# AllenNeuralDynamics/aind-exaspim-image-compression

Hardware: AMD Instinct MI355X
Metric: denoised+encoded voxels/s on 1024^3 uint16 (higher is better)
Workload: dtype f32

## Files before the change

aind-exaspim-image-compression_amd/csrc/stage_kernels.hip:

```cpp
#include <algorithm>
#include <type_traits>

#include "exabm4d_kernels.h"
#include "dct_pairs.h"
#ifdef EXABM4D_STAMPS
#define KERNEL_STAMPS
#endif
#include "kernel_stamps.h"

namespace exabm4d {

typedef float f16v __attribute__((ext_vector_type(16)));

#ifdef EXABM4D_STAMPS
__device__ unsigned long long g_stamps[18];
#endif

constexpr float HAAR_C = 0.70710678118654752440f;

__device__ __forceinline__ void gather8v(__amdgpu_buffer_rsrc_t rsrc, int corner, const unsigned (&voff)[8],
                                         float (&v)[8]) {
#pragma unroll
    for (int y = 0; y < 8; y++)
        v[y] = __int_as_float(__builtin_amdgcn_raw_buffer_load_b32(rsrc, (int)voff[y], corner, 0));
}

template <int K>
__device__ __forceinline__ void haar_fwd2(f2 (&v)[MAXG]) {
#pragma unroll
    for (int len = K; len > 1; len >>= 1) {
        const int half = len >> 1;
        f2 t[MAXG];
#pragma unroll
        for (int i = 0; i < half; i++) {
            t[i] = (v[2 * i] + v[2 * i + 1]) * HAAR_C;
            t[half + i] = (v[2 * i] - v[2 * i + 1]) * HAAR_C;
        }
#pragma unroll
        for (int i = 0; i < len; i++) v[i] = t[i];
    }
}
template <int K>
__device__ __forceinline__ void haar_inv2(f2 (&v)[MAXG]) {
#pragma unroll
    for (int len = 1; len < K; len <<= 1) {
        f2 t[MAXG];
#pragma unroll
        for (int i = 0; i < len; i++) {
            t[2 * i] = (v[i] + v[len + i]) * HAAR_C;
            t[2 * i + 1] = (v[i] - v[len + i]) * HAAR_C;
        }
#pragma unroll
        for (int i = 0; i < 2 * len; i++) v[i] = t[i];
    }
}

typedef unsigned u2v __attribute__((ext_vector_type(2)));
__device__ __forceinline__ void gather8v2(__amdgpu_buffer_rsrc_t rsrc, int corner2, const unsigned (&voff)[8],
                                          float (&a)[8], float (&b)[8]) {
#pragma unroll
    for (int y = 0; y < 8; y++) {
        const u2v t = __builtin_amdgcn_raw_buffer_load_b64(rsrc, (int)(2u * voff[y]), corner2, 0);
        a[y] = __uint_as_float(t.x);
        b[y] = __uint_as_float(t.y);
    }
}

struct TileGeom {
    int y0, x0;
    int nry, nrx;
};

#ifndef EXABM4D_HT_NW
#define EXABM4D_HT_NW 12
#endif
#ifndef EXABM4D_HT_TY
// ... 23 lines not shown
    static constexpr int TBW = 2 * TBUF;
    static constexpr int NW = NW_;
    static constexpr int TY = TY_, TX = TX_;
    static constexpr int ROWS = (TY - 1) * STEP + 18;
    static constexpr int COLS = (TX - 1) * STEP + 18;
    static constexpr int PS = ((ROWS * COLS + 23) / 32) * 32 + 8;
    static constexpr int NPL = NPL_;
    static constexpr size_t LDS_FLOATS = (size_t)2 * NPL * PS + (size_t)NW * TBW + 4 + 2 * NW + 8 + NW;
    static_assert(NW % 2 == 0 && NW <= 16 && NPL >= 18 && NPL <= 26, "pairs of waves; at most 3 layers in flight");
    static_assert(LDS_FLOATS * sizeof(float) <= 160 * 1024, "ring + transpose buffers exceed the CU's LDS");
};
template <bool WIENER>
struct HalfCfg : HalfGeom<EXABM4D_HT_NW, EXABM4D_HT_TY, EXABM4D_HT_TX, EXABM4D_HT_NPL> {};
template <>
struct HalfCfg<true> : HalfGeom<EXABM4D_WIE_NW, EXABM4D_WIE_TY, EXABM4D_WIE_TX, EXABM4D_WIE_NPL> {};
constexpr int HNCNT = 8;
typedef long long ring_t;
constexpr double RINT_MAGIC = 6755399441055744.0;
__device__ __forceinline__ long long magic_bits(double m) {
    const unsigned long long b = (unsigned long long)__double_as_longlong(m);
    const unsigned hi = (unsigned)(b >> 32) - 0x43380000u;
    return (long long)(((unsigned long long)hi << 32) | (b & 0xFFFFFFFFull));
}
#ifndef EXABM4D_WIE_ILV
#define EXABM4D_WIE_ILV 2
#endif
__device__ __forceinline__ f2 rcp_nr2(f2 d) {
    f2 r = mk2(__uint_as_float(0x7EF311C7u - __float_as_uint(d.x)), __uint_as_float(0x7EF311C7u - __float_as_uint(d.y)));
#pragma unroll
    for (int i = 0; i < 3; i++) r = __builtin_elementwise_fma(__builtin_elementwise_fma(-d, r, (f2)(1.0f)), r, r);
    return r;
}
__device__ __forceinline__ f2 wiener_w2(f2 e, float sigma2, unsigned& acc) {
    const f2 W = e * rcp_nr2(e + sigma2);
    const f2 q = __builtin_elementwise_fma(W, W, (f2)(1.0f));
    acc += __float_as_uint(q.x);
    acc += __float_as_uint(q.y);
    return W;
}
constexpr unsigned WSQ_BIAS = 2u * 0x3F800000u;

__device__ __forceinline__ void wait_flag(const int* flag, int want, int lane) {
    cbar();
    if (lane == 0) {
        while (__hip_atomic_load(flag, __ATOMIC_RELAXED, __HIP_MEMORY_SCOPE_WORKGROUP) < want)
            __builtin_amdgcn_s_sleep(4);
    }
    cbar();
}
__device__ __forceinline__ void raise_flag(int* flag, int value, int lane) {
    cbar();
    if (lane == 0) __hip_atomic_store(flag, value, __ATOMIC_RELAXED, __HIP_MEMORY_SCOPE_WORKGROUP);
    cbar();
}

template <int KH>
__device__ __forceinline__ void half_shrink_local(f16v (&S)[4], float thr, int& nnz, f2 (&approx)[4]) {
#pragma unroll
    for (int jp = 0; jp < 4; jp++) {
        f16v A = S[jp];
        f2 x[MAXG];
#pragma unroll
        for (int k = 0; k < KH; k++) x[k] = mk2(A[2 * k], A[2 * k + 1]);
        haar_fwd2<KH>(x);
        approx[jp] = x[0];
#pragma unroll
        for (int k = 1; k < KH; k++) {
            const bool k0 = fabsf(x[k].x) >= thr, k1 = fabsf(x[k].y) >= thr;
            nnz += (k0 ? 1 : 0) + (k1 ? 1 : 0);
            float f0 = k0 ? x[k].x : 0.0f, f1 = k1 ? x[k].y : 0.0f;
            asm volatile("" : "+v"(f0), "+v"(f1));
            A[2 * k] = f0;
            A[2 * k + 1] = f1;
        }
        S[jp] = A;
    }
}
template <int KH>
__device__ __forceinline__ void half_unshrink_local(f16v (&S)[4], const f2 (&approx)[4]) {
#pragma unroll
    for (int jp = 0; jp < 4; jp++) {
        f16v A = S[jp];
        f2 x[MAXG];
        x[0] = approx[jp];
#pragma unroll
        for (int k = 1; k < KH; k++) x[k] = mk2(A[2 * k], A[2 * k + 1]);
        haar_inv2<KH>(x);
#pragma unroll
        for (int k = 0; k < KH; k++) {
            A[2 * k] = x[k].x;
            A[2 * k + 1] = x[k].y;
        }
        S[jp] = A;
    }
}

template <class C>
__device__ __forceinline__ void flush_num_plane(ring_t* ring, long long* __restrict__ num, int z,
                                                const TileGeom& tg, const VolGeom& g, int lane) {
    constexpr int REG = C::COLS;
    ring_t* plane = ring + ((z + 5) % C::NPL) * C::PS;
    constexpr int N = C::ROWS * REG, U = 6;
    const long long e0 = ((long long)z * g.ny + tg.y0) * (long long)g.nx + tg.x0;
    char* const sbase = reinterpret_cast<char*>(num) + e0 * 8;
    constexpr int DQ = 64 / REG, DR = 64 % REG;
    const unsigned row_adj = 8u * (unsigned)(g.nx - REG);
    const unsigned step = 8u * (unsigned)(DQ * g.nx + DR);
    int rxx = lane;
    asm volatile("" : "+v"(rxx));
    unsigned boff = 8u * (unsigned)rxx;
    const int lane0 = rxx;
#pragma unroll
    for (int j = 1; j * REG < 64; j++) {
        const bool w = lane0 >= j * REG;
        rxx -= w ? REG : 0;
        boff += w ? row_adj : 0u;
// ... 24 lines not shown
    int w = lane == 0 ? __hip_atomic_load(lock + 2, __ATOMIC_RELAXED, __HIP_MEMORY_SCOPE_WORKGROUP) : 0;
    w = __builtin_amdgcn_readfirstlane(w);
    if ((w >> 16) == 0) return false;
    {
        const int izp = izb + (w >> 16) - 1;
        if ((w & 0xFFFF) >= grid_pos(izp + 1, g.az, g.nz) - grid_pos(izp, g.az, g.nz)) return false;
    }
    w = lane == 0 ? __hip_atomic_fetch_add(lock + 2, 1, __ATOMIC_RELAXED, __HIP_MEMORY_SCOPE_WORKGROUP) : 0;
    w = __builtin_amdgcn_readfirstlane(w);
    const int gen = w >> 16, i = w & 0xFFFF;
    if (gen == 0) return false;
    const int iz = izb + gen - 1;
    const int z0 = grid_pos(iz, g.az, g.nz), zn = grid_pos(iz + 1, g.az, g.nz);
    if (i >= zn - z0) return false;
    cbar();
    flush_num_plane<C>(ring, num, z0 - RAD + i, tg, g, lane);
    cbar();
    if (lane == 0) __hip_atomic_fetch_add(lock + 3, 1, __ATOMIC_RELAXED, __HIP_MEMORY_SCOPE_WORKGROUP);
    cbar();
    return true;
}

template <int KH>
__device__ __forceinline__ void wiener_half_local(f16v (&S)[4], const f16v (&SB)[4], float sigma2,
                                                  unsigned& sw, f2 (&approx)[8]) {
#pragma unroll
    for (int jp = 0; jp < 4; jp++) {
        f16v A = S[jp];
        const f16v B = SB[jp];
        f2 x[MAXG], y[MAXG];
#pragma unroll
        for (int k = 0; k < KH; k++) {
            x[k] = mk2(A[2 * k], A[2 * k + 1]);
            y[k] = mk2(B[2 * k], B[2 * k + 1]);
        }
        haar_fwd2<KH>(x);
        haar_fwd2<KH>(y);
        approx[jp] = x[0];
        approx[4 + jp] = y[0];
#pragma unroll
        for (int k = 1; k < KH; k++) {
            const f2 W = wiener_w2(y[k] * y[k], sigma2, sw);
            const f2 f = W * x[k];
            A[2 * k] = f.x;
            A[2 * k + 1] = f.y;
            if (EXABM4D_WIE_ILV && (k % EXABM4D_WIE_ILV) == 0) __builtin_amdgcn_sched_barrier(0);
        }
        S[jp] = A;
    }
}

template <bool WIENER, typename TableT>
__device__ __forceinline__ bool process_half_group(
    const float* __restrict__ noisy, const float* __restrict__ basic, const uint32_t* __restrict__ kk,
    int rz, int ry, int rx, const TileGeom& tg, size_t sy, size_t sz, const TableT& T,
    const float (&win)[8], const float* __restrict__ win_g, float thr, float sigma2, double up, ring_t* ring,
    unsigned long long* __restrict__ cvol, f2* tb,
    f2* partner_tb, int* lock, int* sync, int* cnt, int wave, int& seq, int& seen, int layer, int target,
    int lane, long long g_nvox, long long* __restrict__ num, const VolGeom& g, int izb,
    const f2* __restrict__ pair
#ifdef EXABM4D_STAMPS
    , unsigned long long (&st)[16]
#endif
    ) {
    using C = HalfCfg<WIENER>;
    constexpr int HNW = C::NW, HNPL = C::NPL, HPS = C::PS, REG = C::COLS;
    constexpr bool HELP_FLUSH = !WIENER;
    constexpr int NP = WIENER ? 8 : 4;
    const int hi = lane >> 3, lo = lane & 7;
    const int xl = tr_x<WIENER>(hi, lo);
    STAMP(t0);
    const int half = pair_half(wave), partner = wave ^ 1;
    const uint32_t mykey = lane < MAXG ? kk[lane] : KEY_EMPTY;
    const int count = __popcll(__ballot(mykey != KEY_EMPTY));
    int K = 1;
    while (K * 2 <= count) K *= 2;
    const int KH = K > 1 ? K / 2 : 1;
    const int kb = K > 1 ? half * KH : 0;
    const bool active = K > 1 || half == 0;

    int closer = 0;
    auto body = [&](auto KHc) {
        constexpr int KH = decltype(KHc)::value;
        f16v S[4];
        f16v SB[WIENER ? 4 : 1];
#pragma unroll
        for (int j = 0; j < 4; j++) S[j] = (f16v)(0.0f);
        if constexpr (WIENER) {
#pragma unroll
            for (int j = 0; j < 4; j++) SB[j] = (f16v)(0.0f);
        }

        int my_dz, my_dy, my_dx;
        code_to_disp(mykey & KEY_CMASK, my_dz, my_dy, my_dx);
        const unsigned long long my_corner =
            lane < MAXG ? (unsigned long long)(rz + my_dz) * sz +
                              (unsigned long long)(ry + my_dy) * sy + (unsigned long long)(rx + my_dx)
                        : 0ull;
        const int zb = max(rz - RAD, 0);
        const size_t win_off = (size_t)zb * sz;
        const size_t win_left = (size_t)g_nvox - win_off;
        const int win_bytes = (int)min(win_left * sizeof(float), (size_t)0x7FFFFFFFu * 2u);
        const __amdgpu_buffer_rsrc_t noisy_r = __builtin_amdgcn_make_buffer_rsrc(
            const_cast<float*>(noisy + win_off), 0, win_bytes, 0x00020000);
        const __amdgpu_buffer_rsrc_t basic_r = __builtin_amdgcn_make_buffer_rsrc(
            const_cast<float*>((WIENER ? basic : noisy) + win_off), 0, win_bytes, 0x00020000);
        const int my_rel = lane < MAXG ? (int)(4u * (unsigned)(my_corner - win_off)) : 0;
        auto corner_of = [&](int k) -> int { return __builtin_amdgcn_readlane(my_rel, k); };
        const __amdgpu_buffer_rsrc_t pair_r = __builtin_amdgcn_make_buffer_rsrc(
            const_cast<f2*>((WIENER && pair ? pair : reinterpret_cast<const f2*>(noisy)) + (WIENER && pair ? win_off : 0)), 0,
            (int)min(win_left * sizeof(f2), (size_t)0x7FFFFFFFu * 2u), 0x00020000);
        float a[8], b[8];
        f2 v2[8];
        unsigned voff[8];
#pragma unroll
        for (int y = 0; y < 8; y++)
            voff[y] = 4u * ((unsigned)hi * (unsigned)sz + (unsigned)y * (unsigned)sy + (unsigned)lo);
        if constexpr (!WIENER && KH >= 4) {
            float c[8], d[8];
            f2 w2[8];
            gather8v(noisy_r, corner_of(kb), voff, a);
            gather8v(noisy_r, corner_of(kb + 1), voff, b);
            gather8v(noisy_r, corner_of(kb + 2), voff, c);
            gather8v(noisy_r, corner_of(kb + 3), voff, d);
#pragma unroll
            for (int kl = 0; kl < KH; kl += 4) {
#pragma unroll
                for (int j = 0; j < 8; j++) {
                    v2[j] = mk2(a[j], b[j]);
                    w2[j] = mk2(c[j], d[j]);
                }
                if (kl + 4 < KH) {
                    gather8v(noisy_r, corner_of(kb + kl + 4), voff, a);
                    gather8v(noisy_r, corner_of(kb + kl + 5), voff, b);
                    gather8v(noisy_r, corner_of(kb + kl + 6), voff, c);
                    gather8v(noisy_r, corner_of(kb + kl + 7), voff, d);
                }
                pair_fwd_x2<WIENER>(T, tb, hi, lo, v2, w2);
#pragma unroll
                for (int j = 0; j < 8; j++) {
                    S[j >> 1][2 * kl + (j & 1)] = v2[j].x;
                    S[j >> 1][2 * kl + 2 + (j & 1)] = v2[j].y;
                    S[j >> 1][2 * kl + 4 + (j & 1)] = w2[j].x;
                    S[j >> 1][2 * kl + 6 + (j & 1)] = w2[j].y;
                }
            }
        } else if constexpr (!WIENER) {
            gather8v(noisy_r, corner_of(kb), voff, a);
            gather8v(noisy_r, corner_of(kb + (KH > 1 ? 1 : 0)), voff, b);
#pragma unroll
            for (int kl = 0; kl < KH; kl += 2) {
#pragma unroll
                for (int j = 0; j < 8; j++) v2[j] = mk2(a[j], b[j]);
                if (kl + 2 < KH) {
                    gather8v(noisy_r, corner_of(kb + kl + 2), voff, a);
                    gather8v(noisy_r, corner_of(kb + kl + 3), voff, b);
                }
                pair_fwd<WIENER>(T, tb, hi, lo, v2);
#pragma unroll
                for (int j = 0; j < 8; j++) S[j >> 1][2 * kl + (j & 1)] = v2[j].x;
                if constexpr (KH > 1) {
#pragma unroll
                    for (int j = 0; j < 8; j++) S[j >> 1][2 * kl + 2 + (j & 1)] = v2[j].y;
                }
            }
        } else if constexpr (KH == 1) {
            const size_t c0 = corner_of(kb);
            if (pair) {
                gather8v2(pair_r, 2 * (int)c0, voff, a, b);
            } else {
                gather8v(noisy_r, c0, voff, a);
                gather8v(basic_r, c0, voff, b);
            }
#pragma unroll
            for (int j = 0; j < 8; j++) v2[j] = mk2(a[j], b[j]);
            pair_fwd<WIENER>(T, tb, hi, lo, v2);
#pragma unroll
            for (int j = 0; j < 8; j++) {
                S[j >> 1][j & 1] = v2[j].x;
                SB[j >> 1][j & 1] = v2[j].y;
            }
        } else if (pair) {
            gather8v2(pair_r, 2 * corner_of(kb), voff, a, b);
#pragma unroll
            for (int kl = 0; kl < KH; kl++) {
#pragma unroll
                for (int j = 0; j < 8; j++) v2[j] = mk2(a[j], b[j]);
                if (kl + 1 < KH) gather8v2(pair_r, 2 * corner_of(kb + kl + 1), voff, a, b);
                pair_fwd<WIENER>(T, tb, hi, lo, v2);
#pragma unroll
                for (int j = 0; j < 8; j++) {
                    S[j >> 1][2 * kl + (j & 1)] = v2[j].x;
                    SB[j >> 1][2 * kl + (j & 1)] = v2[j].y;
                }
            }
        } else {
            gather8v(noisy_r, corner_of(kb), voff, a);
            gather8v(noisy_r, corner_of(kb + 1), voff, b);
#pragma unroll
            for (int kl = 0; kl < KH; kl += 2) {
#pragma unroll
                for (int j = 0; j < 8; j++) v2[j] = mk2(a[j], b[j]);
                gather8v(basic_r, corner_of(kb + kl), voff, a);
                gather8v(basic_r, corner_of(kb + kl + 1), voff, b);
                pair_fwd<WIENER>(T, tb, hi, lo, v2);
#pragma unroll
                for (int j = 0; j < 8; j++) {
                    S[j >> 1][2 * kl + (j & 1)] = v2[j].x;
                    S[j >> 1][2 * kl + 2 + (j & 1)] = v2[j].y;
                }
#pragma unroll
                for (int j = 0; j < 8; j++) v2[j] = mk2(a[j], b[j]);
                if (kl + 2 < KH) {
                    gather8v(noisy_r, corner_of(kb + kl + 2), voff, a);
                    gather8v(noisy_r, corner_of(kb + kl + 3), voff, b);
                }
                pair_fwd<WIENER>(T, tb, hi, lo, v2);
#pragma unroll
                for (int j = 0; j < 8; j++) {
                    SB[j >> 1][2 * kl + (j & 1)] = v2[j].x;
                    SB[j >> 1][2 * kl + 2 + (j & 1)] = v2[j].y;
                }
            }
        }

        STAMP(t1);
        STAMP_ADD(0, t0, t1);
        int nnz = 0;
        unsigned sw = 0;
        f2 approx[NP];
        if constexpr (WIENER)
            wiener_half_local<KH>(S, SB, sigma2, sw, approx);
        else
            half_shrink_local<KH>(S, thr, nnz, approx);
        f2 top[4];
        if (K > 1) {
            seq++;
#pragma unroll
            for (int jp = 0; jp < NP; jp++) tb[jp * 64 + lane] = approx[jp];
            tb[NP * 64 + lane] = mk2(__int_as_float(WIENER ? (int)sw : nnz), 0.0f);
            raise_flag(sync + wave, seq, lane);
            STAMP(te0);
            wait_flag(sync + partner, seq, lane);
            STAMP(te1);
            STAMP_ADD(2, te0, te1);
            f2 other[NP];
#pragma unroll
            for (int jp = 0; jp < NP; jp++) other[jp] = partner_tb[jp * 64 + lane];
            const float theirs = partner_tb[NP * 64 + lane].x;
            cbar();
            raise_flag(sync + HNW + wave, seq, lane);
            if constexpr (WIENER)
                sw += __float_as_uint(theirs);
            else
                nnz += __float_as_int(theirs);
#pragma unroll
            for (int jp = 0; jp < 4; jp++) {
                const f2 a0 = half ? other[jp] : approx[jp], a1 = half ? approx[jp] : other[jp];
                f2 t0 = (a0 + a1) * HAAR_C, t1 = (a0 - a1) * HAAR_C;
                if constexpr (WIENER) {
                    const f2 b0 = half ? other[4 + jp] : approx[4 + jp];
                    const f2 b1 = half ? approx[4 + jp] : other[4 + jp];
                    const f2 u0 = (b0 + b1) * HAAR_C, u1 = (b0 - b1) * HAAR_C;
                    const f2 W0 = wiener_w2(u0 * u0, sigma2, sw);
                    const f2 W1 = wiener_w2(u1 * u1, sigma2, sw);
                    t0 = W0 * t0;
                    t1 = W1 * t1;
                } else {
                    const bool p0 = fabsf(t0.x) >= thr, p1 = fabsf(t0.y) >= thr;
                    const bool q0 = fabsf(t1.x) >= thr, q1 = fabsf(t1.y) >= thr;
                    nnz += (p0 ? 1 : 0) + (p1 ? 1 : 0) + (q0 ? 1 : 0) + (q1 ? 1 : 0);
                    t0 = mk2(p0 ? t0.x : 0.0f, p1 ? t0.y : 0.0f);
                    t1 = mk2(q0 ? t1.x : 0.0f, q1 ? t1.y : 0.0f);
                }
                top[jp] = half ? (t0 - t1) * HAAR_C : (t0 + t1) * HAAR_C;
                if constexpr (WIENER) __builtin_amdgcn_sched_barrier(0);
            }
        } else {
#pragma unroll
            for (int jp = 0; jp < 4; jp++) {
                if constexpr (WIENER) {
                    const f2 W = wiener_w2(approx[4 + jp] * approx[4 + jp], sigma2, sw);
                    top[jp] = W * approx[jp];
                } else {
                    const bool p0 = fabsf(approx[jp].x) >= thr, p1 = fabsf(approx[jp].y) >= thr;
                    nnz += (p0 ? 1 : 0) + (p1 ? 1 : 0);
                    top[jp] = mk2(p0 ? approx[jp].x : 0.0f, p1 ? approx[jp].y : 0.0f);
                }
            }
        }
        half_unshrink_local<KH>(S, top);
        float w;
        if constexpr (WIENER) {
            sw -= (K > 1 ? 8u * (unsigned)(KH - 1) + 8u : 4u) * WSQ_BIAS;
            unsigned lo16 = sw & 0xFFFFu, hi16 = sw >> 16;
#pragma unroll
            for (int off = 32; off >= 1; off >>= 1) {
                lo16 += __shfl_xor(lo16, off);
                hi16 += __shfl_xor(hi16, off);
            }
            const double q = (double)hi16 * 65536.0 + (double)lo16;
            const float stat = (float)(q * (1.0 / 8388608.0));
            w = 1.0f / (stat > 1.0f ? stat : 1.0f);
        } else {
#pragma unroll
            for (int off = 32; off >= 1; off >>= 1) nnz += __shfl_xor(nnz, off);
            w = 1.0f / (float)(nnz > 1 ? nnz : 1);
        }
        double ww[8];
        if constexpr (WIENER) {
#pragma unroll
            for (int y = 0; y < 8; y++) ww[y] = (double)(w * win_g[(hi * 8 + y) * 8 + xl]) * up;
        } else {
#pragma unroll
// ... 42 lines not shown
                STAMP_ADD(3, tg0, tg1);
            }
        };
        STAMP(t3);
        STAMP_ADD(5, t2, t3);
        auto ring_off = [&](int k) -> int {
            int slot = __builtin_amdgcn_readlane(my_slot0, k) + hi;
            slot -= slot >= HNPL ? HNPL : 0;
            return slot * HPS + __builtin_amdgcn_readlane(my_yx, k) + xl;
        };
        auto ring_add = [&](int off, const f2 (&v)[8], int comp) {
#pragma unroll
            for (int y = 0; y < 8; y++)
                __hip_atomic_fetch_add(reinterpret_cast<unsigned long long*>(ring + off + y * REG),
                                       (unsigned long long)magic_bits(__builtin_fma((double)(comp ? v[y].y : v[y].x), ww[y], RINT_MAGIC)),
                                       __ATOMIC_RELAXED, __HIP_MEMORY_SCOPE_WORKGROUP);
        };
        if constexpr (KH >= 4) {
            f2 w2[8];
#pragma unroll
            for (int kl = 0; kl < KH; kl += 4) {
#pragma unroll
                for (int j = 0; j < 8; j++) {
                    v2[j] = mk2(S[j >> 1][2 * kl + (j & 1)], S[j >> 1][2 * kl + 2 + (j & 1)]);
                    w2[j] = mk2(S[j >> 1][2 * kl + 4 + (j & 1)], S[j >> 1][2 * kl + 6 + (j & 1)]);
                }
                pair_inv_x2<WIENER>(T, tb, hi, lo, v2, w2);
                STAMP(tl1);
                gate(kb + kl);
                ring_add(ring_off(kb + kl), v2, 0);
                gate(kb + kl + 1);
                ring_add(ring_off(kb + kl + 1), v2, 1);
                gate(kb + kl + 2);
                ring_add(ring_off(kb + kl + 2), w2, 0);
                gate(kb + kl + 3);
                ring_add(ring_off(kb + kl + 3), w2, 1);
                STAMP(tl2);
                STAMP_ADD(4, tl1, tl2);
            }
        } else {
#pragma unroll
            for (int kl = 0; kl < KH; kl += 2) {
                constexpr bool two = KH > 1;
                const int kl2 = two ? kl + 1 : kl;
#pragma unroll
                for (int j = 0; j < 8; j++)
                    v2[j] = mk2(S[j >> 1][2 * kl + (j & 1)], S[j >> 1][2 * kl2 + (j & 1)]);
                pair_inv<WIENER>(T, tb, hi, lo, v2);
                STAMP(tl1);
                gate(kb + kl);
                ring_add(ring_off(kb + kl), v2, 0);
                if constexpr (two) {
                    gate(kb + kl2);
                    ring_add(ring_off(kb + kl2), v2, 1);
                }
                STAMP(tl2);
                STAMP_ADD(4, tl1, tl2);
            }
        }
    };
    if (active) {
        switch (KH) {
            case 8: body(std::integral_constant<int, 8>{}); break;
            case 4: body(std::integral_constant<int, 4>{}); break;
            case 2: body(std::integral_constant<int, 2>{}); break;
            default: body(std::integral_constant<int, 1>{}); break;
        }
    }
    if (!active) {
        if (lane == 0) {
            while (__hip_atomic_load(lock + 1, __ATOMIC_RELAXED, __HIP_MEMORY_SCOPE_WORKGROUP) < layer - 2)
                __builtin_amdgcn_s_sleep(8);
        }
        cbar();
    }
    closer = (__hip_atomic_fetch_add(cnt + (layer & (HNCNT - 1)), lane == 0 ? 1 : 0, __ATOMIC_RELAXED,
                                     __HIP_MEMORY_SCOPE_WORKGROUP) + 1 == target) ? 1 : 0;
    return __builtin_amdgcn_readfirstlane(closer) != 0;
}

typedef Dct7 HalfTable;
template <bool WIENER>
__global__ __launch_bounds__(HalfCfg<WIENER>::NW * 64) void stage_half_kernel(
    const float* __restrict__ noisy_all, const float* __restrict__ basic_all,
    const uint32_t* __restrict__ keys_all, VolGeom g, HalfTable T, const float* __restrict__ win_g,
    float thr, float sigma2, const double* __restrict__ qscale, long long* __restrict__ num_all,
    unsigned long long* __restrict__ cvol_all, int tiles_x, int layers_per_chunk, const f2* __restrict__ pair_all,
    int strip) {
    using C = HalfCfg<WIENER>;
    constexpr int HNW = C::NW, HNPL = C::NPL, HPS = C::PS, HTY = C::TY, HTX = C::TX;
    extern __shared__ __align__(16) float lds[];
    ring_t* ring = reinterpret_cast<ring_t*>(lds);
    const int wave = __builtin_amdgcn_readfirstlane(threadIdx.x >> 6), lane = threadIdx.x & 63;
    f2* tb = reinterpret_cast<f2*>(lds + 2 * HNPL * HPS + wave * C::TBW);
    f2* partner_tb = reinterpret_cast<f2*>(lds + 2 * HNPL * HPS + (wave ^ 1) * C::TBW);
    int* lock = reinterpret_cast<int*>(lds + 2 * HNPL * HPS + HNW * C::TBW);
    int* sync = lock + 4;
    int* cnt = sync + 2 * HNW;
    int* pub = cnt + HNCNT;
    int* got = pub + HNW / 2;

    const size_t voff = (size_t)blockIdx.z * (size_t)g.nvox;
    const float* __restrict__ noisy = noisy_all + voff;
    const float* __restrict__ basic = WIENER ? basic_all + voff : nullptr;
    const f2* __restrict__ pair = (WIENER && pair_all) ? pair_all + voff : nullptr;
    long long* __restrict__ num = num_all + voff;
    unsigned long long* __restrict__ cvol = cvol_all + voff;
    const double up = qscale[2 * blockIdx.z];
    const uint32_t* __restrict__ keys = keys_all + (size_t)blockIdx.z * (size_t)g.nref * MAXG;
    const size_t sy = (size_t)g.nx, sz = (size_t)g.nx * (size_t)g.ny;

    const int tile = xcd_contiguous(blockIdx.x, gridDim.x);
    int ty, tx;
    if (strip) {
        const int tiles_y = (int)gridDim.x / tiles_x;
        const int sidx = tile / (strip * tiles_x), r = tile - sidx * (strip * tiles_x);
        const int h = min(strip, tiles_y - sidx * strip);
        tx = r / h;
        ty = sidx * strip + (r - tx * h);
    } else {
        ty = tile / tiles_x;
        tx = tile - ty * tiles_x;
    }
    const int iy0 = HTY * ty, ix0 = HTX * tx;
    TileGeom tg;
    tg.nry = min(HTY, g.gy - iy0);
    tg.nrx = min(HTX, g.gx - ix0);
    tg.y0 = grid_pos(iy0, g.ay, g.ny) - RAD;
// ... 47 lines not shown
            }
            t = __builtin_amdgcn_readfirstlane(t) - 1;
        }
        cbar();
        last = t + 1;
        STAMP(th1);
        STAMP_ADD(6, th0, th1);
        if (t >= total) break;
        const int layer = t / nrefs, r = t - layer * nrefs;
        const int iz = izb + layer;
        const int z0 = grid_pos(iz, g.az, g.nz);
        const int jy = r / tg.nrx, jx = r - jy * tg.nrx;
        const int iy = iy0 + jy, ix = ix0 + jx;
        const int ry = grid_pos(iy, g.ay, g.ny), rx = grid_pos(ix, g.ax, g.nx);
        const uint32_t* kk = keys + ((size_t)((size_t)iz * g.gy + iy) * g.gx + ix) * MAXG;
        {
            int f = __hip_atomic_load(lock + 1, __ATOMIC_RELAXED, __HIP_MEMORY_SCOPE_WORKGROUP);
            f = __builtin_amdgcn_readfirstlane(f);
            if (layer <= f)
                __builtin_amdgcn_s_setprio(1);
            else
                __builtin_amdgcn_s_setprio(0);
        }
        const bool closer = process_half_group<WIENER>(
            noisy, basic, kk, z0, ry, rx, tg, sy, sz, tab, win, win_g, thr, sigma2, up, ring, cvol, tb,
            partner_tb, lock, sync, cnt, wave, seq, seen, layer, 2 * nrefs, lane, g.nvox, num, g, izb, pair
#ifdef EXABM4D_STAMPS
            , st
#endif
        );
        if (closer) {
            STAMP(tc0);
            if (lane == 0)
                __hip_atomic_store(cnt + (layer & (HNCNT - 1)), 0, __ATOMIC_RELAXED,
                                   __HIP_MEMORY_SCOPE_WORKGROUP);
            if (lane == 0) {
                while (__hip_atomic_load(lock + 1, __ATOMIC_RELAXED,
                                         __HIP_MEMORY_SCOPE_WORKGROUP) != layer)
                    __builtin_amdgcn_s_sleep(2);
            }
            cbar();
            if (iz + 1 < ize) {
                const int zn = grid_pos(iz + 1, g.az, g.nz);
                if constexpr (!WIENER) {
                    if (lane == 0) {
                        __hip_atomic_store(lock + 3, 0, __ATOMIC_RELAXED, __HIP_MEMORY_SCOPE_WORKGROUP);
                        __hip_atomic_store(lock + 2, (layer + 1) << 16, __ATOMIC_RELAXED,
// ... 26 lines not shown
    }
#ifdef EXABM4D_STAMPS
    st[7] = stamp() - tk0;
    if (lane == 0)
        for (int i = 0; i < 9; i++) atomicAdd(&g_stamps[i + (WIENER ? 9 : 0)], st[i]);
#endif
}

__global__ __launch_bounds__(256) void interleave_pair_kernel(const float* __restrict__ a, const float* __restrict__ b,
                                                              f2* __restrict__ out, size_t n) {
    for (size_t i = ((size_t)blockIdx.x * 256 + threadIdx.x) * 4; i < n; i += (size_t)gridDim.x * 1024) {
        if (i + 4 <= n) {
            const f4 x = *reinterpret_cast<const f4*>(a + i), y = *reinterpret_cast<const f4*>(b + i);
            f4 lo, hi;
            lo.x = x.x; lo.y = y.x; lo.z = x.y; lo.w = y.y;
            hi.x = x.z; hi.y = y.z; hi.z = x.w; hi.w = y.w;
            *reinterpret_cast<f4*>(out + i) = lo;
            *reinterpret_cast<f4*>(out + i + 2) = hi;
        } else {
            for (size_t j = i; j < n; j++) out[j] = mk2(a[j], b[j]);
        }
    }
}
hipError_t launch_stage(const float* noisy, const float* basic, const uint32_t* keys,
                        const VolGeom& g, int batch, const float* dct64, const float* win_dev,
                        float thr, float sigma2, const double* qscale, long long* num,
                        unsigned long long* cw, hipStream_t stream, const StageOpts& opt, float* pair,
                        int pair_ready) {
    DctTable T;
    for (int i = 0; i < 64; i++) T.d[i] = dct64[i];
    const size_t n = (size_t)g.nvox * (size_t)batch;
    Dct7 HT;
    if (!make_dct7(T, HT)) return hipErrorInvalidValue;
    auto launch = [&](auto wiener_c) -> hipError_t {
        constexpr bool W = decltype(wiener_c)::value;
        using C = HalfCfg<W>;
        if (((unsigned long long)(C::ROWS - 1) * (unsigned long long)g.nx + C::COLS) * 8ull > 0xFFFFFFFFull)
            return hipErrorInvalidValue;
        const int hty =(g.gy + C::TY - 1) / C::TY, htx = (g.gx + C::TX - 1) / C::TX;
        const long long htiles = (long long)hty * htx * batch;
        int hchunks = (int)((1024 + htiles - 1) / htiles);
        const int fine = (int)std::min<long long>((32768 + htiles - 1) / htiles, g.gz / 16);
        if (hchunks < fine) hchunks = fine;
        if (opt.chunks > 0) hchunks = opt.chunks;
        if (hchunks < 1) hchunks = 1;
        if (hchunks > g.gz) hchunks = g.gz;
        const int hlpc = (g.gz + hchunks - 1) / hchunks;
        hchunks = (g.gz + hlpc - 1) / hlpc;
        const dim3 hgrid((unsigned)(hty * htx), (unsigned)hchunks, (unsigned)batch);
        const size_t lds = sizeof(float) * C::LDS_FLOATS;
        hipError_t err = hipFuncSetAttribute(reinterpret_cast<const void*>(&stage_half_kernel<W>),
                                             hipFuncAttributeMaxDynamicSharedMemorySize, (int)lds);
        if (err != hipSuccess) return err;
        const f2* pairvol = nullptr;
        const bool vec_ok = (n % 4) == 0 && (((uintptr_t)noisy | (uintptr_t)basic) & 15u) == 0;
        if (W && pair && opt.pairvol && (pair_ready || vec_ok)) {
            f2* pv = reinterpret_cast<f2*>(pair);
            if (!pair_ready)
                hipLaunchKernelGGL(interleave_pair_kernel, dim3(65536), dim3(256), 0, stream, noisy, basic, pv, n);
            pairvol = pv;
        }
        hipLaunchKernelGGL(stage_half_kernel<W>, hgrid, dim3(C::NW * 64), lds, stream, noisy, basic, keys,
                           g, HT, win_dev, thr, sigma2, qscale, num, cw, htx, hlpc, pairvol, opt.strip);
        return hipGetLastError();
    };
    return basic ? launch(std::true_type{}) : launch(std::false_type{});
}

#ifdef EXABM4D_STAMPS
extern "C" void exabm4d_debug_stamps(unsigned long long* out, int reset) {
    unsigned long long z[18] = {};
    (void)hipDeviceSynchronize();
    (void)hipMemcpyFromSymbol(out, HIP_SYMBOL(g_stamps), sizeof(z));
    if (reset) (void)hipMemcpyToSymbol(HIP_SYMBOL(g_stamps), z, sizeof(z));
}
#endif

}
```

Before: 2.024 billion.

## Fuse first Haar level into gather and keep group coefficients in f2 pairs

Replaces the f16v-based group storage and generic Haar forward/inverse loops with per-row f2 arrays. The first Haar level is applied as soon as each transformed patch pair is produced, and the remaining levels use packed v_pk_add_f32 butterflies with op_sel/neg_hi in inline asm. It also splits the Wiener kernel into pair-volume and separate-volume template instantiations, so the pair check becomes compile-time and the separate-volume path gathers noisy and basic per neighbor. The goal is fewer register shuffles and ALU ops in the grouped 1D transform, at the cost of hand-written asm and more code paths.

```diff
diff --git a/aind-exaspim-image-compression_amd/csrc/stage_kernels.hip b/aind-exaspim-image-compression_amd/csrc/stage_kernels.hip
--- a/aind-exaspim-image-compression_amd/csrc/stage_kernels.hip
+++ b/aind-exaspim-image-compression_amd/csrc/stage_kernels.hip
@@ -10,7 +10,6 @@
 
 namespace exabm4d {
 
-typedef float f16v __attribute__((ext_vector_type(16)));
 
 #ifdef EXABM4D_STAMPS
 __device__ unsigned long long g_stamps[18];
@@ -25,33 +24,58 @@
         v[y] = __int_as_float(__builtin_amdgcn_raw_buffer_load_b32(rsrc, (int)voff[y], corner, 0));
 }
 
-template <int K>
-__device__ __forceinline__ void haar_fwd2(f2 (&v)[MAXG]) {
-#pragma unroll
-    for (int len = K; len > 1; len >>= 1) {
-        const int half = len >> 1;
-        f2 t[MAXG];
-#pragma unroll
-        for (int i = 0; i < half; i++) {
-            t[i] = (v[2 * i] + v[2 * i + 1]) * HAAR_C;
-            t[half + i] = (v[2 * i] - v[2 * i + 1]) * HAAR_C;
-        }
-#pragma unroll
-        for (int i = 0; i < len; i++) v[i] = t[i];
-    }
-}
-template <int K>
-__device__ __forceinline__ void haar_inv2(f2 (&v)[MAXG]) {
-#pragma unroll
-    for (int len = 1; len < K; len <<= 1) {
-        f2 t[MAXG];
-#pragma unroll
-        for (int i = 0; i < len; i++) {
-            t[2 * i] = (v[i] + v[len + i]) * HAAR_C;
-            t[2 * i + 1] = (v[i] - v[len + i]) * HAAR_C;
-        }
-#pragma unroll
-        for (int i = 0; i < 2 * len; i++) v[i] = t[i];
+template <int SA, int SB>
+__device__ __forceinline__ f2 bfly(f2 a, f2 b) {
+    f2 r;
+    if constexpr (SA == 0 && SB == 0)
+        asm("v_pk_add_f32 %0, %1, %2 op_sel:[0,0] op_sel_hi:[0,0] neg_hi:[0,1]" : "=v"(r) : "v"(a), "v"(b));
+    else if constexpr (SA == 0 && SB == 1)
+        asm("v_pk_add_f32 %0, %1, %2 op_sel:[0,1] op_sel_hi:[0,1] neg_hi:[0,1]" : "=v"(r) : "v"(a), "v"(b));
+    else if constexpr (SA == 1 && SB == 0)
+        asm("v_pk_add_f32 %0, %1, %2 op_sel:[1,0] op_sel_hi:[1,0] neg_hi:[0,1]" : "=v"(r) : "v"(a), "v"(b));
+    else
+        asm("v_pk_add_f32 %0, %1, %2 op_sel:[1,1] op_sel_hi:[1,1] neg_hi:[0,1]" : "=v"(r) : "v"(a), "v"(b));
+    return r;
+}
+__device__ __forceinline__ f2 bfly_sel(int sa, int sb, f2 a, f2 b) {
+    return sa ? (sb ? bfly<1, 1>(a, b) : bfly<1, 0>(a, b)) : (sb ? bfly<0, 1>(a, b) : bfly<0, 0>(a, b));
+}
+__device__ __forceinline__ f2 haar_l1(f2 v) { return bfly<0, 1>(v, v) * HAAR_C; }
+constexpr int haar_pairs(int KH) { return KH > 1 ? KH / 2 : 1; }
+template <int KH, class F>
+__device__ __forceinline__ void haar_fwd_upper(f2 (&q)[haar_pairs(KH)], F&& det) {
+    if constexpr (KH >= 4) {
+#pragma unroll
+        for (int i = 0; i < KH / 4; i++) {
+            const f2 r = bfly<0, 0>(q[2 * i], q[2 * i + 1]) * HAAR_C;
+            const float d0 = det(q[2 * i].y), d1 = det(q[2 * i + 1].y);
+            q[2 * i + 1] = mk2(d0, d1);
+            q[2 * i] = r;
+        }
+    }
+    if constexpr (KH == 8) {
+        const f2 r = bfly<0, 0>(q[0], q[2]) * HAAR_C;
+        const float d0 = det(q[0].y), d1 = det(q[2].y);
+        q[2] = mk2(d0, d1);
+        q[0] = r;
+    }
+}
+template <int KH>
+__device__ __forceinline__ void haar_inv_lower(f2 (&q)[haar_pairs(KH)], f2 a) {
+    if constexpr (KH == 2) {
+        q[0] = a;
+    } else if constexpr (KH == 4) {
+        const f2 p0 = bfly<0, 0>(a, q[1]) * HAAR_C, p1 = bfly<1, 1>(a, q[1]) * HAAR_C;
+        q[0] = p0;
+        q[1] = p1;
+    } else {
+        const f2 v0 = bfly<0, 0>(a, q[2]) * HAAR_C, v1 = bfly<1, 1>(a, q[2]) * HAAR_C;
+        const f2 p0 = bfly<0, 0>(v0, q[1]) * HAAR_C, p1 = bfly<1, 1>(v0, q[1]) * HAAR_C;
+        const f2 p2 = bfly<0, 0>(v1, q[3]) * HAAR_C, p3 = bfly<1, 1>(v1, q[3]) * HAAR_C;
+        q[0] = p0;
+        q[1] = p1;
+        q[2] = p2;
+        q[3] = p3;
     }
 }
 
@@ -121,9 +145,6 @@
     const unsigned hi = (unsigned)(b >> 32) - 0x43380000u;
     return (long long)(((unsigned long long)hi << 32) | (b & 0xFFFFFFFFull));
 }
-#ifndef EXABM4D_WIE_ILV
-#define EXABM4D_WIE_ILV 2
-#endif
 __device__ __forceinline__ f2 rcp_nr2(f2 d) {
     f2 r = mk2(__uint_as_float(0x7EF311C7u - __float_as_uint(d.x)), __uint_as_float(0x7EF311C7u - __float_as_uint(d.y)));
 #pragma unroll
@@ -153,44 +174,19 @@
     cbar();
 }
 
+__device__ __forceinline__ float ht_keep(float v, float thr, int& nnz) {
+    const bool k = fabsf(v) >= thr;
+    nnz += k ? 1 : 0;
+    float f = k ? v : 0.0f;
+    asm volatile("" : "+v"(f));
+    return f;
+}
 template <int KH>
-__device__ __forceinline__ void half_shrink_local(f16v (&S)[4], float thr, int& nnz, f2 (&approx)[4]) {
-#pragma unroll
-    for (int jp = 0; jp < 4; jp++) {
-        f16v A = S[jp];
-        f2 x[MAXG];
-#pragma unroll
-        for (int k = 0; k < KH; k++) x[k] = mk2(A[2 * k], A[2 * k + 1]);
-        haar_fwd2<KH>(x);
-        approx[jp] = x[0];
-#pragma unroll
-        for (int k = 1; k < KH; k++) {
-            const bool k0 = fabsf(x[k].x) >= thr, k1 = fabsf(x[k].y) >= thr;
-            nnz += (k0 ? 1 : 0) + (k1 ? 1 : 0);
-            float f0 = k0 ? x[k].x : 0.0f, f1 = k1 ? x[k].y : 0.0f;
-            asm volatile("" : "+v"(f0), "+v"(f1));
-            A[2 * k] = f0;
-            A[2 * k + 1] = f1;
-        }
-        S[jp] = A;
-    }
-}
-template <int KH>
-__device__ __forceinline__ void half_unshrink_local(f16v (&S)[4], const f2 (&approx)[4]) {
-#pragma unroll
-    for (int jp = 0; jp < 4; jp++) {
-        f16v A = S[jp];
-        f2 x[MAXG];
-        x[0] = approx[jp];
-#pragma unroll
-        for (int k = 1; k < KH; k++) x[k] = mk2(A[2 * k], A[2 * k + 1]);
-        haar_inv2<KH>(x);
-#pragma unroll
-        for (int k = 0; k < KH; k++) {
-            A[2 * k] = x[k].x;
-            A[2 * k + 1] = x[k].y;
-        }
-        S[jp] = A;
+__device__ __forceinline__ void half_shrink_local(f2 (&X)[8][haar_pairs(KH)], float thr, int& nnz) {
+#pragma unroll
+    for (int j = 0; j < 8; j++) {
+        haar_fwd_upper<KH>(X[j], [&](float v) { return ht_keep(v, thr, nnz); });
+        if constexpr (KH > 1) X[j][0].y = ht_keep(X[j][0].y, thr, nnz);
     }
 }
 
@@ -261,35 +257,29 @@
 }
 
 template <int KH>
-__device__ __forceinline__ void wiener_half_local(f16v (&S)[4], const f16v (&SB)[4], float sigma2,
-                                                  unsigned& sw, f2 (&approx)[8]) {
-#pragma unroll
-    for (int jp = 0; jp < 4; jp++) {
-        f16v A = S[jp];
-        const f16v B = SB[jp];
-        f2 x[MAXG], y[MAXG];
-#pragma unroll
-        for (int k = 0; k < KH; k++) {
-            x[k] = mk2(A[2 * k], A[2 * k + 1]);
-            y[k] = mk2(B[2 * k], B[2 * k + 1]);
-        }
-        haar_fwd2<KH>(x);
-        haar_fwd2<KH>(y);
-        approx[jp] = x[0];
-        approx[4 + jp] = y[0];
-#pragma unroll
-        for (int k = 1; k < KH; k++) {
-            const f2 W = wiener_w2(y[k] * y[k], sigma2, sw);
-            const f2 f = W * x[k];
-            A[2 * k] = f.x;
-            A[2 * k + 1] = f.y;
-            if (EXABM4D_WIE_ILV && (k % EXABM4D_WIE_ILV) == 0) __builtin_amdgcn_sched_barrier(0);
-        }
-        S[jp] = A;
-    }
-}
-
-template <bool WIENER, typename TableT>
+__device__ __forceinline__ void wiener_half_local(f2 (&X)[8][haar_pairs(KH)], f2 (&Y)[8][haar_pairs(KH)],
+                                                  float sigma2, unsigned& sw) {
+    auto same = [](float v) { return v; };
+#pragma unroll
+    for (int j = 0; j < 8; j++) {
+        haar_fwd_upper<KH>(X[j], same);
+        haar_fwd_upper<KH>(Y[j], same);
+#pragma unroll
+        for (int m = 1; m < haar_pairs(KH); m++) {
+            const f2 W = wiener_w2(Y[j][m] * Y[j][m], sigma2, sw);
+            X[j][m] = W * X[j][m];
+        }
+        if constexpr (KH > 1) {
+            if (j & 1) {
+                const f2 W = wiener_w2(mk2(Y[j - 1][0].y * Y[j - 1][0].y, Y[j][0].y * Y[j][0].y), sigma2, sw);
+                X[j - 1][0].y = W.x * X[j - 1][0].y;
+                X[j][0].y = W.y * X[j][0].y;
+            }
+        }
+    }
+}
+
+template <bool WIENER, bool SEPVOL, typename TableT>
 __device__ __forceinline__ bool process_half_group(
     const float* __restrict__ noisy, const float* __restrict__ basic, const uint32_t* __restrict__ kk,
     int rz, int ry, int rx, const TileGeom& tg, size_t sy, size_t sz, const TableT& T,
@@ -306,6 +296,7 @@
     constexpr int HNW = C::NW, HNPL = C::NPL, HPS = C::PS, REG = C::COLS;
     constexpr bool HELP_FLUSH = !WIENER;
     constexpr int NP = WIENER ? 8 : 4;
+    constexpr bool PAIRVOL = WIENER && !SEPVOL;
     const int hi = lane >> 3, lo = lane & 7;
     const int xl = tr_x<WIENER>(hi, lo);
     STAMP(t0);
@@ -321,14 +312,9 @@
     int closer = 0;
     auto body = [&](auto KHc) {
         constexpr int KH = decltype(KHc)::value;
-        f16v S[4];
-        f16v SB[WIENER ? 4 : 1];
-#pragma unroll
-        for (int j = 0; j < 4; j++) S[j] = (f16v)(0.0f);
-        if constexpr (WIENER) {
-#pragma unroll
-            for (int j = 0; j < 4; j++) SB[j] = (f16v)(0.0f);
-        }
+        constexpr int HP = haar_pairs(KH);
+        f2 X[8][HP];
+        f2 Y[WIENER ? 8 : 1][HP];
 
         int my_dz, my_dy, my_dx;
         code_to_disp(mykey & KEY_CMASK, my_dz, my_dy, my_dx);
@@ -347,7 +333,7 @@
         const int my_rel = lane < MAXG ? (int)(4u * (unsigned)(my_corner - win_off)) : 0;
         auto corner_of = [&](int k) -> int { return __builtin_amdgcn_readlane(my_rel, k); };
         const __amdgpu_buffer_rsrc_t pair_r = __builtin_amdgcn_make_buffer_rsrc(
-            const_cast<f2*>((WIENER && pair ? pair : reinterpret_cast<const f2*>(noisy)) + (WIENER && pair ? win_off : 0)), 0,
+            const_cast<f2*>((PAIRVOL ? pair : reinterpret_cast<const f2*>(noisy)) + (PAIRVOL ? win_off : 0)), 0,
             (int)min(win_left * sizeof(f2), (size_t)0x7FFFFFFFu * 2u), 0x00020000);
         float a[8], b[8];
         f2 v2[8];
@@ -378,10 +364,8 @@
                 pair_fwd_x2<WIENER>(T, tb, hi, lo, v2, w2);
 #pragma unroll
                 for (int j = 0; j < 8; j++) {
-                    S[j >> 1][2 * kl + (j & 1)] = v2[j].x;
-                    S[j >> 1][2 * kl + 2 + (j & 1)] = v2[j].y;
-                    S[j >> 1][2 * kl + 4 + (j & 1)] = w2[j].x;
-                    S[j >> 1][2 * kl + 6 + (j & 1)] = w2[j].y;
+                    X[j][kl / 2] = haar_l1(v2[j]);
+                    X[j][kl / 2 + 1] = haar_l1(w2[j]);
                 }
             }
         } else if constexpr (!WIENER) {
@@ -397,15 +381,11 @@
                 }
                 pair_fwd<WIENER>(T, tb, hi, lo, v2);
 #pragma unroll
-                for (int j = 0; j < 8; j++) S[j >> 1][2 * kl + (j & 1)] = v2[j].x;
-                if constexpr (KH > 1) {
-#pragma unroll
-                    for (int j = 0; j < 8; j++) S[j >> 1][2 * kl + 2 + (j & 1)] = v2[j].y;
-                }
+                for (int j = 0; j < 8; j++) X[j][kl / 2] = KH > 1 ? haar_l1(v2[j]) : v2[j];
             }
         } else if constexpr (KH == 1) {
             const size_t c0 = corner_of(kb);
-            if (pair) {
+            if constexpr (PAIRVOL) {
                 gather8v2(pair_r, 2 * (int)c0, voff, a, b);
             } else {
                 gather8v(noisy_r, c0, voff, a);
@@ -416,50 +396,46 @@
             pair_fwd<WIENER>(T, tb, hi, lo, v2);
 #pragma unroll
             for (int j = 0; j < 8; j++) {
-                S[j >> 1][j & 1] = v2[j].x;
-                SB[j >> 1][j & 1] = v2[j].y;
-            }
-        } else if (pair) {
-            gather8v2(pair_r, 2 * corner_of(kb), voff, a, b);
+                X[j][0] = v2[j];
+                Y[j][0] = mk2(v2[j].y, v2[j].y);
+            }
+        } else {
+            f2 ab[8];
+            auto gather_nb = [&](int k) {
+                if constexpr (PAIRVOL) {
+                    const int c2 = 2 * corner_of(k);
+#pragma unroll
+                    for (int y = 0; y < 8; y++) {
+                        const u2v t = __builtin_amdgcn_raw_buffer_load_b64(pair_r, (int)(2u * voff[y]), c2, 0);
+                        ab[y] = mk2(__uint_as_float(t.x), __uint_as_float(t.y));
+                    }
+                } else {
+                    const int c = corner_of(k);
+#pragma unroll
+                    for (int y = 0; y < 8; y++)
+                        ab[y] = mk2(__int_as_float(__builtin_amdgcn_raw_buffer_load_b32(noisy_r, (int)voff[y], c, 0)),
+                                    __int_as_float(__builtin_amdgcn_raw_buffer_load_b32(basic_r, (int)voff[y], c, 0)));
+                }
+            };
+            gather_nb(kb);
+            f2 z0[8];
 #pragma unroll
             for (int kl = 0; kl < KH; kl++) {
 #pragma unroll
-                for (int j = 0; j < 8; j++) v2[j] = mk2(a[j], b[j]);
-                if (kl + 1 < KH) gather8v2(pair_r, 2 * corner_of(kb + kl + 1), voff, a, b);
+                for (int j = 0; j < 8; j++) v2[j] = ab[j];
+                if (kl + 1 < KH) gather_nb(kb + kl + 1);
                 pair_fwd<WIENER>(T, tb, hi, lo, v2);
-#pragma unroll
-                for (int j = 0; j < 8; j++) {
-                    S[j >> 1][2 * kl + (j & 1)] = v2[j].x;
-                    SB[j >> 1][2 * kl + (j & 1)] = v2[j].y;
-                }
-            }
-        } else {
-            gather8v(noisy_r, corner_of(kb), voff, a);
-            gather8v(noisy_r, corner_of(kb + 1), voff, b);
-#pragma unroll
-            for (int kl = 0; kl < KH; kl += 2) {
-#pragma unroll
-                for (int j = 0; j < 8; j++) v2[j] = mk2(a[j], b[j]);
-                gather8v(basic_r, corner_of(kb + kl), voff, a);
-                gather8v(basic_r, corner_of(kb + kl + 1), voff, b);
-                pair_fwd<WIENER>(T, tb, hi, lo, v2);
-#pragma unroll
-                for (int j = 0; j < 8; j++) {
-                    S[j >> 1][2 * kl + (j & 1)] = v2[j].x;
-                    S[j >> 1][2 * kl + 2 + (j & 1)] = v2[j].y;
-                }
-#pragma unroll
-                for (int j = 0; j < 8; j++) v2[j] = mk2(a[j], b[j]);
-                if (kl + 2 < KH) {
-                    gather8v(noisy_r, corner_of(kb + kl + 2), voff, a);
-                    gather8v(noisy_r, corner_of(kb + kl + 3), voff, b);
-                }
-                pair_fwd<WIENER>(T, tb, hi, lo, v2);
-#pragma unroll
-                for (int j = 0; j < 8; j++) {
-                    SB[j >> 1][2 * kl + (j & 1)] = v2[j].x;
-                    SB[j >> 1][2 * kl + 2 + (j & 1)] = v2[j].y;
-                }
+                if ((kl & 1) == 0) {
+#pragma unroll
+                    for (int j = 0; j < 8; j++) z0[j] = v2[j];
+                } else {
+#pragma unroll
+                    for (int j = 0; j < 8; j++) {
+                        X[j][kl / 2] = bfly<0, 0>(z0[j], v2[j]) * HAAR_C;
+                        Y[j][kl / 2] = bfly<1, 1>(z0[j], v2[j]) * HAAR_C;
+                    }
+                }
+                __builtin_amdgcn_sched_barrier(0);
             }
         }
 
@@ -467,25 +443,33 @@
         STAMP_ADD(0, t0, t1);
         int nnz = 0;
         unsigned sw = 0;
-        f2 approx[NP];
         if constexpr (WIENER)
-            wiener_half_local<KH>(S, SB, sigma2, sw, approx);
+            wiener_half_local<KH>(X, Y, sigma2, sw);
         else
-            half_shrink_local<KH>(S, thr, nnz, approx);
-        f2 top[4];
-        if (K > 1) {
+            half_shrink_local<KH>(X, thr, nnz);
+        const unsigned smask = half ? 0x80000000u : 0u;
+        if (KH > 1 || K > 1) {
             seq++;
-#pragma unroll
-            for (int jp = 0; jp < NP; jp++) tb[jp * 64 + lane] = approx[jp];
+            float* const tbf = reinterpret_cast<float*>(tb);
+#pragma unroll
+            for (int j = 0; j < 8; j++) {
+                tbf[(j >> 1) * 128 + 2 * lane + (j & 1)] = X[j][0].x;
+                if constexpr (WIENER) tbf[(4 + (j >> 1)) * 128 + 2 * lane + (j & 1)] = Y[j][0].x;
+            }
             tb[NP * 64 + lane] = mk2(__int_as_float(WIENER ? (int)sw : nnz), 0.0f);
             raise_flag(sync + wave, seq, lane);
             STAMP(te0);
             wait_flag(sync + partner, seq, lane);
             STAMP(te1);
             STAMP_ADD(2, te0, te1);
-            f2 other[NP];
-#pragma unroll
-            for (int jp = 0; jp < NP; jp++) other[jp] = partner_tb[jp * 64 + lane];
+            const f2* const tb_lo = half ? partner_tb : tb;
+            const f2* const tb_hi = half ? tb : partner_tb;
+            f2 first[NP], second[NP];
+#pragma unroll
+            for (int jp = 0; jp < NP; jp++) {
+                first[jp] = tb_lo[jp * 64 + lane];
+                second[jp] = tb_hi[jp * 64 + lane];
+            }
             const float theirs = partner_tb[NP * 64 + lane].x;
             cbar();
             raise_flag(sync + HNW + wave, seq, lane);
@@ -495,40 +479,45 @@
                 nnz += __float_as_int(theirs);
 #pragma unroll
             for (int jp = 0; jp < 4; jp++) {
-                const f2 a0 = half ? other[jp] : approx[jp], a1 = half ? approx[jp] : other[jp];
-                f2 t0 = (a0 + a1) * HAAR_C, t1 = (a0 - a1) * HAAR_C;
+                f2 t[2], u[2];
+#pragma unroll
+                for (int c = 0; c < 2; c++) {
+                    t[c] = bfly_sel(c, c, first[jp], second[jp]);
+                    if constexpr (WIENER) u[c] = bfly_sel(c, c, first[4 + jp], second[4 + jp]);
+                }
+#pragma unroll
+                for (int c = 0; c < 2; c++) {
+                    f2 tt = t[c] * HAAR_C;
+                    if constexpr (WIENER) {
+                        const f2 uu = u[c] * HAAR_C;
+                        tt = wiener_w2(uu * uu, sigma2, sw) * tt;
+                    } else {
+                        const float k0 = ht_keep(tt.x, thr, nnz), k1 = ht_keep(tt.y, thr, nnz);
+                        tt = mk2(k0, k1);
+                    }
+                    X[2 * jp + c][0].x = (tt.x + __uint_as_float(__float_as_uint(tt.y) ^ smask)) * HAAR_C;
+                }
+                if constexpr (WIENER) __builtin_amdgcn_sched_barrier(0);
+            }
+        } else {
+#pragma unroll
+            for (int jp = 0; jp < 4; jp++) {
+                const float x0 = X[2 * jp][0].x, x1 = X[2 * jp + 1][0].x;
                 if constexpr (WIENER) {
-                    const f2 b0 = half ? other[4 + jp] : approx[4 + jp];
-                    const f2 b1 = half ? approx[4 + jp] : other[4 + jp];
-                    const f2 u0 = (b0 + b1) * HAAR_C, u1 = (b0 - b1) * HAAR_C;
-                    const f2 W0 = wiener_w2(u0 * u0, sigma2, sw);
-                    const f2 W1 = wiener_w2(u1 * u1, sigma2, sw);
-                    t0 = W0 * t0;
-                    t1 = W1 * t1;
+                    const float y0 = Y[2 * jp][0].x, y1 = Y[2 * jp + 1][0].x;
+                    const f2 W = wiener_w2(mk2(y0 * y0, y1 * y1), sigma2, sw);
+                    X[2 * jp][0].x = W.x * x0;
+                    X[2 * jp + 1][0].x = W.y * x1;
                 } else {
-                    const bool p0 = fabsf(t0.x) >= thr, p1 = fabsf(t0.y) >= thr;
-                    const bool q0 = fabsf(t1.x) >= thr, q1 = fabsf(t1.y) >= thr;
-                    nnz += (p0 ? 1 : 0) + (p1 ? 1 : 0) + (q0 ? 1 : 0) + (q1 ? 1 : 0);
-                    t0 = mk2(p0 ? t0.x : 0.0f, p1 ? t0.y : 0.0f);
-                    t1 = mk2(q0 ? t1.x : 0.0f, q1 ? t1.y : 0.0f);
-                }
-                top[jp] = half ? (t0 - t1) * HAAR_C : (t0 + t1) * HAAR_C;
-                if constexpr (WIENER) __builtin_amdgcn_sched_barrier(0);
-            }
-        } else {
-#pragma unroll
-            for (int jp = 0; jp < 4; jp++) {
-                if constexpr (WIENER) {
-                    const f2 W = wiener_w2(approx[4 + jp] * approx[4 + jp], sigma2, sw);
-                    top[jp] = W * approx[jp];
-                } else {
-                    const bool p0 = fabsf(approx[jp].x) >= thr, p1 = fabsf(approx[jp].y) >= thr;
-                    nnz += (p0 ? 1 : 0) + (p1 ? 1 : 0);
-                    top[jp] = mk2(p0 ? approx[jp].x : 0.0f, p1 ? approx[jp].y : 0.0f);
-                }
-            }
-        }
-        half_unshrink_local<KH>(S, top);
+                    X[2 * jp][0].x = ht_keep(x0, thr, nnz);
+                    X[2 * jp + 1][0].x = ht_keep(x1, thr, nnz);
+                }
+            }
+        }
+        if constexpr (KH > 1) {
+#pragma unroll
+            for (int j = 0; j < 8; j++) haar_inv_lower<KH>(X[j], haar_l1(X[j][0]));
+        }
         float w;
         if constexpr (WIENER) {
             sw -= (K > 1 ? 8u * (unsigned)(KH - 1) + 8u : 4u) * WSQ_BIAS;
@@ -617,8 +606,8 @@
             for (int kl = 0; kl < KH; kl += 4) {
 #pragma unroll
                 for (int j = 0; j < 8; j++) {
-                    v2[j] = mk2(S[j >> 1][2 * kl + (j & 1)], S[j >> 1][2 * kl + 2 + (j & 1)]);
-                    w2[j] = mk2(S[j >> 1][2 * kl + 4 + (j & 1)], S[j >> 1][2 * kl + 6 + (j & 1)]);
+                    v2[j] = X[j][kl / 2];
+                    w2[j] = X[j][kl / 2 + 1];
                 }
                 pair_inv_x2<WIENER>(T, tb, hi, lo, v2, w2);
                 STAMP(tl1);
@@ -639,8 +628,7 @@
                 constexpr bool two = KH > 1;
                 const int kl2 = two ? kl + 1 : kl;
 #pragma unroll
-                for (int j = 0; j < 8; j++)
-                    v2[j] = mk2(S[j >> 1][2 * kl + (j & 1)], S[j >> 1][2 * kl2 + (j & 1)]);
+                for (int j = 0; j < 8; j++) v2[j] = two ? X[j][kl / 2] : mk2(X[j][0].x, X[j][0].x);
                 pair_inv<WIENER>(T, tb, hi, lo, v2);
                 STAMP(tl1);
                 gate(kb + kl);
@@ -675,10 +663,10 @@
 }
 
 typedef Dct7 HalfTable;
-template <bool WIENER>
-__global__ __launch_bounds__(HalfCfg<WIENER>::NW * 64) void stage_half_kernel(
+template <bool WIENER, bool SEPVOL>
+__device__ __forceinline__ void stage_half_body(
     const float* __restrict__ noisy_all, const float* __restrict__ basic_all,
-    const uint32_t* __restrict__ keys_all, VolGeom g, HalfTable T, const float* __restrict__ win_g,
+    const uint32_t* __restrict__ keys_all, const VolGeom& g, const HalfTable& T, const float* __restrict__ win_g,
     float thr, float sigma2, const double* __restrict__ qscale, long long* __restrict__ num_all,
     unsigned long long* __restrict__ cvol_all, int tiles_x, int layers_per_chunk, const f2* __restrict__ pair_all,
     int strip) {
@@ -698,7 +686,7 @@
     const size_t voff = (size_t)blockIdx.z * (size_t)g.nvox;
     const float* __restrict__ noisy = noisy_all + voff;
     const float* __restrict__ basic = WIENER ? basic_all + voff : nullptr;
-    const f2* __restrict__ pair = (WIENER && pair_all) ? pair_all + voff : nullptr;
+    const f2* __restrict__ pair = (WIENER && !SEPVOL) ? pair_all + voff : nullptr;
     long long* __restrict__ num = num_all + voff;
     unsigned long long* __restrict__ cvol = cvol_all + voff;
     const double up = qscale[2 * blockIdx.z];
@@ -792,7 +780,7 @@
             else
                 __builtin_amdgcn_s_setprio(0);
         }
-        const bool closer = process_half_group<WIENER>(
+        const bool closer = process_half_group<WIENER, SEPVOL>(
             noisy, basic, kk, z0, ry, rx, tg, sy, sz, tab, win, win_g, thr, sigma2, up, ring, cvol, tb,
             partner_tb, lock, sync, cnt, wave, seq, seen, layer, 2 * nrefs, lane, g.nvox, num, g, izb, pair
 #ifdef EXABM4D_STAMPS
@@ -865,6 +853,26 @@
         }
     }
 }
+template <bool WIENER>
+__global__ __launch_bounds__(HalfCfg<WIENER>::NW * 64) void stage_half_kernel(
+    const float* __restrict__ noisy_all, const float* __restrict__ basic_all,
+    const uint32_t* __restrict__ keys_all, VolGeom g, HalfTable T, const float* __restrict__ win_g,
+    float thr, float sigma2, const double* __restrict__ qscale, long long* __restrict__ num_all,
+    unsigned long long* __restrict__ cvol_all, int tiles_x, int layers_per_chunk, const f2* __restrict__ pair_all,
+    int strip) {
+    stage_half_body<WIENER, false>(noisy_all, basic_all, keys_all, g, T, win_g, thr, sigma2, qscale, num_all, cvol_all,
+                                   tiles_x, layers_per_chunk, pair_all, strip);
+}
+__global__ __launch_bounds__(HalfCfg<true>::NW * 64) void stage_half_sep_kernel(
+    const float* __restrict__ noisy_all, const float* __restrict__ basic_all,
+    const uint32_t* __restrict__ keys_all, VolGeom g, HalfTable T, const float* __restrict__ win_g,
+    float thr, float sigma2, const double* __restrict__ qscale, long long* __restrict__ num_all,
+    unsigned long long* __restrict__ cvol_all, int tiles_x, int layers_per_chunk, const f2* __restrict__ pair_all,
+    int strip) {
+    stage_half_body<true, true>(noisy_all, basic_all, keys_all, g, T, win_g, thr, sigma2, qscale, num_all, cvol_all,
+                                tiles_x, layers_per_chunk, pair_all, strip);
+}
+
 hipError_t launch_stage(const float* noisy, const float* basic, const uint32_t* keys,
                         const VolGeom& g, int batch, const float* dct64, const float* win_dev,
                         float thr, float sigma2, const double* qscale, long long* num,
@@ -892,9 +900,6 @@
         hchunks = (g.gz + hlpc - 1) / hlpc;
         const dim3 hgrid((unsigned)(hty * htx), (unsigned)hchunks, (unsigned)batch);
         const size_t lds = sizeof(float) * C::LDS_FLOATS;
-        hipError_t err = hipFuncSetAttribute(reinterpret_cast<const void*>(&stage_half_kernel<W>),
-                                             hipFuncAttributeMaxDynamicSharedMemorySize, (int)lds);
-        if (err != hipSuccess) return err;
         const f2* pairvol = nullptr;
         const bool vec_ok = (n % 4) == 0 && (((uintptr_t)noisy | (uintptr_t)basic) & 15u) == 0;
         if (W && pair && opt.pairvol && (pair_ready || vec_ok)) {
@@ -903,7 +908,11 @@
                 hipLaunchKernelGGL(interleave_pair_kernel, dim3(65536), dim3(256), 0, stream, noisy, basic, pv, n);
             pairvol = pv;
         }
-        hipLaunchKernelGGL(stage_half_kernel<W>, hgrid, dim3(C::NW * 64), lds, stream, noisy, basic, keys,
+        auto* kern = (W && !pairvol) ? &stage_half_sep_kernel : &stage_half_kernel<W>;
+        hipError_t err = hipFuncSetAttribute(reinterpret_cast<const void*>(kern),
+                                             hipFuncAttributeMaxDynamicSharedMemorySize, (int)lds);
+        if (err != hipSuccess) return err;
+        hipLaunchKernelGGL(kern, hgrid, dim3(C::NW * 64), lds, stream, noisy, basic, keys,
                            g, HT, win_dev, thr, sigma2, qscale, num, cw, htx, hlpc, pairvol, opt.strip);
         return hipGetLastError();
     };
```

Measured after the change: 2.046 billion, median of 6. 1.1% higher.
